# qiujiaming315/edgeml-object-detection

Hardware: AMD Instinct MI355X
Metric: images/sec/GPU at 640x640 (SSDLite & FRCNN-R50); ORIE max-abs-diff vs ref (higher is better)
Workload: dtype f32; 1 GPU; ssdlite320_mobilenet_v3_large b=32 640x640 (configs[1]); global_batch=32, parallelism=dp1, batches_in_flight=4, conv_math=bf16x6, weights=seeded synthetic (COCO weights need a download)

## Files before the change

### edgeml-object-detection_amd/csrc/layers.hip

```cpp
#include <cmath>
#include <cstdlib>
#include <mutex>
#include <type_traits>
#include <utility>
#include <vector>

#include "kernels.hpp"

namespace edgedet {



__device__ __forceinline__ float div_fast(float a, float b, float rb) {
    const float q = a * rb;
    return fmaf(fmaf(-q, b, a), rb, q);
}

template <typename T, bool FAST = false>
__device__ __forceinline__ float pre_load(const T* src, int64_t i) {
    if constexpr (sizeof(T) == 1) return FAST ? div_fast((float)src[i], 255.f, 1.f / 255.f) : (float)src[i] / 255.f;
    else return src[i];
}

template <typename T, bool FAST = false>
__device__ __forceinline__ f32x4 pre_pixel(const T* __restrict__ xb, int H, int W, float sh, float sw,
                                           const float* mean, const float* stdv, const float* rstd, int oy, int ox) {
    float ry = __builtin_fmaf(sh, (float)oy + 0.5f, -0.5f);
    float rx = __builtin_fmaf(sw, (float)ox + 0.5f, -0.5f);
    ry = ry < 0.f ? 0.f : ry;
    rx = rx < 0.f ? 0.f : rx;
    const int y0 = min((int)ry, H - 1), x0 = min((int)rx, W - 1);
    const int y1 = y0 + ((y0 < H - 1) ? 1 : 0);
    const int x1 = x0 + ((x0 < W - 1) ? 1 : 0);
    const float ly = fminf(fmaxf(ry - (float)y0, 0.f), 1.f), lx = fminf(fmaxf(rx - (float)x0, 0.f), 1.f);
    const float hy = 1.f - ly, hx = 1.f - lx;
    float v[3];
#pragma unroll
    for (int c = 0; c < 3; ++c) {
        const T* src = xb + (int64_t)c * H * W;
        auto norm = [&](int64_t i) {
            const float a = pre_load<T, FAST>(src, i) - mean[c];
            return FAST ? div_fast(a, stdv[c], rstd[c]) : a / stdv[c];
        };
        const float a00 = norm((int64_t)y0 * W + x0);
        const float a01 = norm((int64_t)y0 * W + x1);
        const float a10 = norm((int64_t)y1 * W + x0);
        const float a11 = norm((int64_t)y1 * W + x1);
        v[c] = __builtin_fmaf(__builtin_fmaf(a00, hx, a01 * lx), hy, __builtin_fmaf(a10, hx, a11 * lx) * ly);
    }
    return f32x4{v[0], v[1], v[2], 0.f};
}

static bool u8_fast_div(const float mean[3], const float stdv[3], float rstd[3]) {
    const float r255 = 1.f / 255.f;
    for (int c = 0; c < 3; ++c) rstd[c] = 1.f / stdv[c];
    auto same = [](float a, float b) { return __builtin_memcmp(&a, &b, sizeof(float)) == 0; };
    auto fast = [](float a, float b, float rb) {
        const float q = a * rb;
        return std::fma(std::fma(-q, b, a), rb, q);
    };
    for (int x = 0; x < 256; ++x) {
        const float xf = (float)x, t = xf / 255.f;
        if (!same(fast(xf, 255.f, r255), t)) return false;
        for (int c = 0; c < 3; ++c) {
            const float a = t - mean[c];
            if (!same(fast(a, stdv[c], rstd[c]), a / stdv[c])) return false;
        }
    }
    return true;
}

template <typename T, bool FAST>
__global__ void preprocess_kernel(PreParams p, const T* __restrict__ x) {
    const int64_t idx = (int64_t)blockIdx.x * blockDim.x + threadIdx.x;
    const int64_t total = (int64_t)p.B * p.Hp * p.Wp;
    if (idx >= total) return;
    const int ox = (int)(idx % p.Wp);
    const int oy = (int)((idx / p.Wp) % p.Hp);
    const int b = (int)(idx / ((int64_t)p.Wp * p.Hp));
    f32x4 out = {0.f, 0.f, 0.f, 0.f};
    if (oy < p.Ho && ox < p.Wo) out = pre_pixel<T, FAST>(x + (int64_t)b * 3 * p.H * p.W, p.H, p.W, p.sh, p.sw, p.mean, p.stdv, p.rstd, oy, ox);
    *reinterpret_cast<f32x4*>(p.y + idx * 4) = out;
}

int preprocess_launch(const PreParams& p0, hipStream_t s) {
    PreParams p = p0;
    EDGEDET_REQUIRE(p.y && ((p.x != nullptr) != (p.xu8 != nullptr)), "preprocess: null y, or not exactly one of x (f32) / x (u8)");
    EDGEDET_REQUIRE(p.Hp >= p.Ho && p.Wp >= p.Wo && p.Ho > 0 && p.Wo > 0, "preprocess: bad sizes");
    p.sh = (float)p.H / (float)p.Ho;
    p.sw = (float)p.W / (float)p.Wo;
    const int64_t total = (int64_t)p.B * p.Hp * p.Wp;
    p.fastdiv = p.xu8 && u8_fast_div(p.mean, p.stdv, p.rstd);
    if (p.xu8) {
        void (*k)(PreParams, const uint8_t*) = p.fastdiv ? preprocess_kernel<uint8_t, true> : preprocess_kernel<uint8_t, false>;
        hipLaunchKernelGGL(k, dim3((unsigned)cdiv(total, 256)), dim3(256), 0, s, p, p.xu8);
    } else {
        void (*k)(PreParams, const float*) = preprocess_kernel<float, false>;
        hipLaunchKernelGGL(k, dim3((unsigned)cdiv(total, 256)), dim3(256), 0, s, p, p.x);
    }
    EDGEDET_LAUNCH_CHECK();
    return 0;
}


__global__ void dwconv_kernel(DwParams p) {
    const int C4 = p.C >> 2;
    const int64_t idx = (int64_t)blockIdx.x * blockDim.x + threadIdx.x;
    const int64_t total = (int64_t)p.B * p.Ho * p.Wo * C4;
    if (idx >= total) return;
    const int c = (int)(idx % C4) * 4;
    const int64_t pix = idx / C4;
    const int ow = (int)(pix % p.Wo);
    const int oh = (int)((pix / p.Wo) % p.Ho);
    const int b = (int)(pix / ((int64_t)p.Wo * p.Ho));
    const float* xb = p.x + (int64_t)b * p.H * p.W * p.C + c;
    f32x4 acc = {0.f, 0.f, 0.f, 0.f};
    const int ih0 = oh * p.stride - p.pad, iw0 = ow * p.stride - p.pad;
    for (int kh = 0; kh < p.K; ++kh) {
        const int ih = ih0 + kh;
        if ((unsigned)ih >= (unsigned)p.H) continue;
        for (int kw = 0; kw < p.K; ++kw) {
            const int iw = iw0 + kw;
            if ((unsigned)iw >= (unsigned)p.W) continue;
            const f32x4 xv = *reinterpret_cast<const f32x4*>(xb + ((int64_t)ih * p.W + iw) * p.C);
            const f32x4 wv = *reinterpret_cast<const f32x4*>(p.w + (kh * p.K + kw) * p.C + c);
            acc.x = fmaf(xv.x, wv.x, acc.x);
            acc.y = fmaf(xv.y, wv.y, acc.y);
            acc.z = fmaf(xv.z, wv.z, acc.z);
            acc.w = fmaf(xv.w, wv.w, acc.w);
        }
    }
    const f32x4 bv = *reinterpret_cast<const f32x4*>(p.bias + c);
    f32x4 o;
    o.x = apply_act(acc.x + bv.x, p.act);
    o.y = apply_act(acc.y + bv.y, p.act);
    o.z = apply_act(acc.z + bv.z, p.act);
    o.w = apply_act(acc.w + bv.w, p.act);
    *reinterpret_cast<f32x4*>(p.y + pix * p.C + c) = o;
}

__global__ void __launch_bounds__(256) dwconv_se_kernel(DwParams p) {
    __shared__ f32x4 red[16][16];
    const int cq = threadIdx.x & 15, pl = threadIdx.x >> 4;
    const int c = blockIdx.x * 64 + cq * 4;
    const int sidx = blockIdx.y, b = blockIdx.z;
    const int HWo = p.Ho * p.Wo;
    const int p0 = (int)((int64_t)sidx * HWo / p.parts), p1 = (int)((int64_t)(sidx + 1) * HWo / p.parts);
    f32x4 sum = {0.f, 0.f, 0.f, 0.f};
    if (c < p.C) {
        const float* xb = p.x + (int64_t)b * p.H * p.W * p.C + c;
        const f32x4 bv = *reinterpret_cast<const f32x4*>(p.bias + c);
        for (int pix = p0 + pl; pix < p1; pix += 16) {
            const int oh = pix / p.Wo, ow = pix - oh * p.Wo;
            const int ih0 = oh * p.stride - p.pad, iw0 = ow * p.stride - p.pad;
            f32x4 acc = {0.f, 0.f, 0.f, 0.f};
            for (int kh = 0; kh < p.K; ++kh) {
                const int ih = ih0 + kh;
                if ((unsigned)ih >= (unsigned)p.H) continue;
                for (int kw = 0; kw < p.K; ++kw) {
                    const int iw = iw0 + kw;
                    if ((unsigned)iw >= (unsigned)p.W) continue;
                    const f32x4 xv = *reinterpret_cast<const f32x4*>(xb + ((int64_t)ih * p.W + iw) * p.C);
                    const f32x4 wv = *reinterpret_cast<const f32x4*>(p.w + (kh * p.K + kw) * p.C + c);
                    acc.x = fmaf(xv.x, wv.x, acc.x);
                    acc.y = fmaf(xv.y, wv.y, acc.y);
                    acc.z = fmaf(xv.z, wv.z, acc.z);
                    acc.w = fmaf(xv.w, wv.w, acc.w);
                }
            }
            f32x4 o;
            o.x = apply_act(acc.x + bv.x, p.act);
            o.y = apply_act(acc.y + bv.y, p.act);
            o.z = apply_act(acc.z + bv.z, p.act);
            o.w = apply_act(acc.w + bv.w, p.act);
            *reinterpret_cast<f32x4*>(p.y + ((int64_t)b * HWo + pix) * p.C + c) = o;
            sum += o;
        }
    }
    red[pl][cq] = sum;
    __syncthreads();
    if (pl == 0 && c < p.C) {
        f32x4 t = red[0][cq];
        for (int q = 1; q < 16; ++q) t += red[q][cq];
        *reinterpret_cast<f32x4*>(p.part + ((int64_t)b * p.parts + sidx) * p.C + c) = t;
    }
}

template <int K, int S>
constexpr int dw_rows() {
    return K == 5 && S == 2 ? 2 : 3;
}

template <int K, int S, int PW>
__device__ __forceinline__ void dw_cols(const DwParams& p, uint32_t lane, int iw0, uint32_t (&co)[(PW - 1) * S + K]) {
    const int cb = p.C * 4, hi = (p.W - 1) * cb;
    int o = iw0 * cb;
#pragma unroll
    for (int j = 0; j < (PW - 1) * S + K; ++j, o += cb) co[j] = lane + (uint32_t)min(max(o, 0), hi);
}

template <int K, int S, int PW>
__device__ __forceinline__ void dw_load_row(const DwParams& p, const float* __restrict__ base,
                                            const uint32_t (&co)[(PW - 1) * S + K], int ih,
                                            f32x4 (&x)[(PW - 1) * S + K]) {
    const uint32_t ro = (uint32_t)(min(max(ih, 0), p.H - 1) * p.W) * (uint32_t)(p.C * 4);
#pragma unroll
    for (int j = 0; j < (PW - 1) * S + K; ++j)
        x[j] = *reinterpret_cast<const f32x4*>(reinterpret_cast<const char*>(base) + (co[j] + ro));
}

template <int K, int S, int PW, typename WF>
__device__ __forceinline__ void dw_fma_row(const DwParams& p, int ih, int iw0, f32x4 (&x)[(PW - 1) * S + K], WF w,
                                           f32x4 (&acc)[PW]) {
    const bool rin = (unsigned)ih < (unsigned)p.H;
#pragma unroll
    for (int j = 0; j < (PW - 1) * S + K; ++j)
        x[j] = rin && (unsigned)(iw0 + j) < (unsigned)p.W ? x[j] : f32x4{0.f, 0.f, 0.f, 0.f};
    f32x4 wv[K];
#pragma unroll
    for (int kw = 0; kw < K; ++kw) wv[kw] = w(kw);
#pragma unroll
    for (int kw = 0; kw < K; ++kw)
#pragma unroll
        for (int o = 0; o < PW; ++o) acc[o] = __builtin_elementwise_fma(x[o * S + kw], wv[kw], acc[o]);
}

template <int PW, bool SUM, typename AF>
__device__ __forceinline__ void dw_store(const DwParams& p, float* yb, int ow0, const f32x4 (&acc)[PW],
                                         const f32x4& bv, f32x4& sum, AF af) {
#pragma unroll
    for (int o = 0; o < PW; ++o) {
        if (ow0 + o < p.Wo) {
            f32x4 v;
            v.x = af(acc[o].x + bv.x);
            v.y = af(acc[o].y + bv.y);
            v.z = af(acc[o].z + bv.z);
            v.w = af(acc[o].w + bv.w);
            *reinterpret_cast<f32x4*>(yb + (int64_t)o * p.C) = v;
            if (SUM) sum += v;
        }
    }
}

template <int PW, bool SUM>
__device__ __forceinline__ void dw_finish(const DwParams& p, float* yb, int ow0, const f32x4 (&acc)[PW],
                                          const f32x4& bv, f32x4& sum) {
    const int act = p.act;
    if (act == ACT_HSWISH)
        dw_store<PW, SUM>(p, yb, ow0, acc, bv, sum, [](float v) { return apply_act(v, ACT_HSWISH); });
    else if (act == ACT_RELU)
        dw_store<PW, SUM>(p, yb, ow0, acc, bv, sum, [](float v) { return apply_act(v, ACT_RELU); });
    else if (act == ACT_NONE)
        dw_store<PW, SUM>(p, yb, ow0, acc, bv, sum, [](float v) { return apply_act(v, ACT_NONE); });
    else
        dw_store<PW, SUM>(p, yb, ow0, acc, bv, sum, [act](float v) { return apply_act(v, act); });
}

template <int K, int S, int PW>
__device__ __forceinline__ void dwconv_rb_body(const DwParams& p, int nq, int nwg, int64_t idx) {
    constexpr int IW = (PW - 1) * S + K;
    const int64_t total = (int64_t)p.B * p.Ho * nwg * nq;
    if (idx >= total) return;
    int q, wg, oh, b;
    if (total <= 0x7fffffff) {
        const uint32_t i = (uint32_t)idx, r0 = i / (uint32_t)nq, r1 = r0 / (uint32_t)nwg;
        q = (int)(i - r0 * (uint32_t)nq);
        wg = (int)(r0 - r1 * (uint32_t)nwg);
        b = (int)(r1 / (uint32_t)p.Ho);
        oh = (int)(r1 - (uint32_t)b * (uint32_t)p.Ho);
    } else {
        q = (int)(idx % nq);
        int64_t r = idx / nq;
        wg = (int)(r % nwg);
        r /= nwg;
        oh = (int)(r % p.Ho);
        b = (int)(r / p.Ho);
    }
    constexpr int R = dw_rows<K, S>();
    const int c = q * 4, ow0 = wg * PW;
    const int ih0 = oh * S - p.pad, iw0 = ow0 * S - p.pad;
    const float* wq = p.w + c;
    uint32_t co[IW];
    dw_cols<K, S, PW>(p, ((uint32_t)(b * p.H * p.W) * (uint32_t)p.C + (uint32_t)c) * 4u, iw0, co);
    f32x4 buf[R][IW], wr[R][K], acc[PW];
#pragma unroll
    for (int r = 0; r < R; ++r) {
        dw_load_row<K, S, PW>(p, p.x, co, ih0 + r, buf[r]);
#pragma unroll
        for (int kw = 0; kw < K; ++kw) wr[r][kw] = *reinterpret_cast<const f32x4*>(wq + (r * K + kw) * p.C);
    }
    const f32x4 bv = *reinterpret_cast<const f32x4*>(p.bias + c);
#pragma unroll
    for (int o = 0; o < PW; ++o) acc[o] = f32x4{0.f, 0.f, 0.f, 0.f};
#pragma unroll
    for (int kh = 0; kh < K; ++kh) {
        const int sl = kh % R;
        dw_fma_row<K, S, PW>(p, ih0 + kh, iw0, buf[sl], [&](int kw) { return wr[sl][kw]; }, acc);
        if (kh + R < K) {
            dw_load_row<K, S, PW>(p, p.x, co, ih0 + kh + R, buf[sl]);
#pragma unroll
            for (int kw = 0; kw < K; ++kw)
                wr[sl][kw] = *reinterpret_cast<const f32x4*>(wq + ((kh + R) * K + kw) * p.C);
        }
    }
    f32x4 unused;
    dw_finish<PW, false>(p, p.y + (((int64_t)b * p.Ho + oh) * p.Wo + ow0) * p.C + c, ow0, acc, bv, unused);
}

template <int K, int S, int PW>
__global__ void __launch_bounds__(256) dwconv_rb_kernel(DwParams p, int nq, int nwg) {
    dwconv_rb_body<K, S, PW>(p, nq, nwg, (int64_t)blockIdx.x * blockDim.x + threadIdx.x);
}

template <int K, int S, int PW>
__global__ void __launch_bounds__(256) dwconv_rb_group_kernel(DwGroup g) {
    const int bx = (int)blockIdx.x;
    int k = 0;
    while (k + 1 < g.n && bx >= g.start[k + 1]) ++k;
    dwconv_rb_body<K, S, PW>(g.p[k], g.nq[k], g.nwg[k], (int64_t)(bx - g.start[k]) * blockDim.x + threadIdx.x);
}

template <int K, int S>
constexpr int dw_se_waves() {
    return K == 3 && S == 2 ? 2 : 3;
}

template <int K, int S, int PW, int QL = 16>
__global__ void __launch_bounds__(256, (dw_se_waves<K, S>())) dwconv_rb_se_kernel(DwParams p, int nq, int nwg) {
    constexpr int GL = 256 / QL;
    constexpr int IW = (PW - 1) * S + K, R = dw_rows<K, S>();
    __shared__ f32x4 red[GL][QL];
    constexpr int WU = ((K * K + 1) * QL + 255) / 256;
    __shared__ f32x4 wl[WU * GL][QL];
    const int ql = threadIdx.x % QL, gl = threadIdx.x / QL;
    const int q = blockIdx.x * QL + ql;
    const int c = q * 4;
    const int sidx = blockIdx.y, b = blockIdx.z;
    const int G = p.Ho * nwg;
    const int g0 = (int)((int64_t)sidx * G / p.parts), g1 = (int)((int64_t)(sidx + 1) * G / p.parts);
    const bool live = q < nq;
    const int cl = live ? c : (nq - 1) * 4;
    const float* xb = p.x + (int64_t)b * p.H * p.W * p.C;
    f32x4 sum = {0.f, 0.f, 0.f, 0.f};
    f32x4 buf[R][IW];
    int g = g0 + gl;
    if (live && g < g1) {
        const int oh = g / nwg, ow0 = (g - oh * nwg) * PW;
        uint32_t co[IW];
        dw_cols<K, S, PW>(p, (uint32_t)cl * 4u, ow0 * S - p.pad, co);
#pragma unroll
        for (int r = 0; r < R; ++r) dw_load_row<K, S, PW>(p, xb, co, oh * S - p.pad + r, buf[r]);
    }
    {
        f32x4 wv[WU];
        const int tq = min(q, nq - 1) * 4;
#pragma unroll
        for (int u = 0; u < WU; ++u) {
            const int t = gl + u * GL;
            wv[u] = *reinterpret_cast<const f32x4*>((t < K * K ? p.w + t * p.C : p.bias) + tq);
        }
#pragma unroll
        for (int u = 0; u < WU; ++u) wl[gl + u * GL][ql] = wv[u];
    }
    __syncthreads();
    auto pass = [&](auto more) {
        constexpr bool MORE = decltype(more)::value;
        const int oh = g / nwg, ow0 = (g - oh * nwg) * PW;
        const int ih0 = oh * S - p.pad, iw0 = ow0 * S - p.pad;
        const int gn = g + GL;
        const int ohn = gn / nwg, ih0n = ohn * S - p.pad, iw0n = (gn - ohn * nwg) * PW * S - p.pad;
        int qv = ql;
        asm volatile("" : "+v"(qv));
        f32x4 acc[PW];
#pragma unroll
        for (int o = 0; o < PW; ++o) acc[o] = f32x4{0.f, 0.f, 0.f, 0.f};
#pragma unroll
        for (int kh = 0; kh < K; ++kh) {
            const int sl = kh % R;
            dw_fma_row<K, S, PW>(p, ih0 + kh, iw0, buf[sl], [&](int kw) { return wl[kh * K + kw][qv]; }, acc);
            if (kh + R < K || MORE) {
                const bool own = kh + R < K;
                uint32_t co[IW];
                dw_cols<K, S, PW>(p, (uint32_t)cl * 4u, own ? iw0 : iw0n, co);
                dw_load_row<K, S, PW>(p, xb, co, own ? ih0 + kh + R : ih0n + sl, buf[sl]);
            }
        }
        dw_finish<PW, true>(p, p.y + (((int64_t)b * p.Ho + oh) * p.Wo + ow0) * p.C + c, ow0, acc, wl[K * K][qv], sum);
        g = gn;
    };
    if (live && g < g1) {
        while (g + GL < g1) pass(std::true_type{});
        pass(std::false_type{});
    }
    red[gl][ql] = sum;
    __syncthreads();
    if (gl == 0 && live) {
        f32x4 t = red[0][ql];
        for (int k = 1; k < GL; ++k) t += red[k][ql];
        *reinterpret_cast<f32x4*>(p.part + ((int64_t)b * p.parts + sidx) * p.C + c) = t;
    }
}

static bool dw_offsets_fit(const DwParams& p) { return (int64_t)p.B * p.H * p.W * p.C * 4 < (1ll << 31); }

template <int K, int S>
static int dwconv_rb_launch(const DwParams& p, hipStream_t s) {
    constexpr int PW = 4;
    const int nq = p.C / 4, nwg = cdiv(p.Wo, PW);
    if (p.part) {
        hipLaunchKernelGGL((dwconv_rb_se_kernel<K, S, PW>), dim3((unsigned)cdiv(nq, 16), p.parts, p.B), dim3(256), 0,
                           s, p, nq, nwg);
    } else {
        const int64_t total = (int64_t)p.B * p.Ho * nwg * nq;
        hipLaunchKernelGGL((dwconv_rb_kernel<K, S, PW>), dim3((unsigned)cdiv(total, 256)), dim3(256), 0, s, p, nq,
                           nwg);
    }
    EDGEDET_LAUNCH_CHECK();
    return 0;
}

constexpr int STEM_T = 16, STEM_SH = STEM_T + 2, STEM_XH = 2 * STEM_SH + 1, STEM_SS = 20;
constexpr int STEM_W0 = 0, STEM_B0 = 576, STEM_WD = 592, STEM_BD = 736, STEM_W1 = 752, STEM_B1 = 1008, STEM_NW = 1024;

template <typename T, bool FUSED, bool FAST = false>
__global__ void __launch_bounds__(256) ssd_stem_kernel(StemParams p, int tiles_w) {
    __shared__ __attribute__((aligned(16))) float xs[STEM_XH * STEM_XH * 4];
    __shared__ __attribute__((aligned(16))) float ss[STEM_SH * STEM_SH * STEM_SS];
    __shared__ __attribute__((aligned(16))) float ws[STEM_NW];
    const int tid = threadIdx.x, b = blockIdx.y;
    const int oh0 = (blockIdx.x / tiles_w) * STEM_T, ow0 = (blockIdx.x % tiles_w) * STEM_T;
    const int sh0 = oh0 - 1, sw0 = ow0 - 1;
    const int xh0 = 2 * sh0 - 1, xw0 = 2 * sw0 - 1;
    const float* xb = FUSED ? nullptr : p.x + (int64_t)b * p.H * p.W * 4;
    {
        float wv[STEM_NW / 256];
#pragma unroll
        for (int r = 0; r < STEM_NW / 256; ++r) {
            const int e = tid + 256 * r;
            const float* src = e < STEM_B0   ? p.w0 + (e / 36) * p.ld0 + e % 36
                               : e < STEM_WD ? p.b0 + (e - STEM_B0)
                               : e < STEM_BD ? p.wd + (e - STEM_WD)
                               : e < STEM_W1 ? p.bd + (e - STEM_BD)
                               : e < STEM_B1 ? p.w1 + ((e - STEM_W1) / 16) * p.ld1 + (e - STEM_W1) % 16
                                             : p.b1 + (e - STEM_B1);
            wv[r] = *src;
        }
        constexpr int R = (STEM_XH * STEM_XH + 255) / 256;
        f32x4 xv[R];
#pragma unroll
        for (int r = 0; r < R; ++r) {
            const int v = tid + 256 * r;
            const int ih = xh0 + v / STEM_XH, iw = xw0 + v % STEM_XH;
            const bool in = v < STEM_XH * STEM_XH && (unsigned)ih < (unsigned)p.H && (unsigned)iw < (unsigned)p.W;
            if constexpr (FUSED) {
                const T* img = (const T*)(sizeof(T) == 1 ? (const void*)p.src8 : (const void*)p.src) +
                               (int64_t)b * 3 * p.H0 * p.W0;
                xv[r] = in ? pre_pixel<T, FAST>(img, p.H0, p.W0, p.sh, p.sw, p.mean, p.stdv, p.rstd, ih, iw)
                           : f32x4{0.f, 0.f, 0.f, 0.f};
            } else {
                const float* src = xb + (in ? ((int64_t)ih * p.W + iw) * 4 : 0);
                xv[r] = *reinterpret_cast<const f32x4*>(src);
                if (!in) xv[r] = f32x4{0.f, 0.f, 0.f, 0.f};
            }
        }
#pragma unroll
        for (int r = 0; r < R; ++r)
            if (tid + 256 * r < STEM_XH * STEM_XH) *reinterpret_cast<f32x4*>(xs + 4 * (tid + 256 * r)) = xv[r];
#pragma unroll
        for (int r = 0; r < STEM_NW / 256; ++r) ws[tid + 256 * r] = wv[r];
    }
    __syncthreads();
    const int lane = tid & 63, wid = tid >> 6, l16 = lane & 15, q4 = lane >> 4;
    float wb[9];
#pragma unroll
    for (int t = 0; t < 9; ++t) wb[t] = ws[STEM_W0 + l16 * 36 + 4 * t + q4];
    const float b0v = ws[STEM_B0 + l16];
    constexpr int NV = STEM_SH * STEM_SH, NTL = (NV + 15) / 16;
    for (int tl = wid; tl < NTL; tl += 4) {
        const int va = min(16 * tl + l16, NV - 1);
        const int lh = va / STEM_SH, lw = va - lh * STEM_SH;
        f32x4 acc = {0.f, 0.f, 0.f, 0.f};
#pragma unroll
        for (int t = 0; t < 9; ++t) {
            const float av = xs[4 * ((2 * lh + t / 3) * STEM_XH + 2 * lw + t % 3) + q4];
            acc = __builtin_amdgcn_mfma_f32_16x16x4f32(av, wb[t], acc, 0, 0, 0);
        }
#pragma unroll
        for (int i = 0; i < 4; ++i) {
            const int v = 16 * tl + 4 * q4 + i;
            if (v < NV) {
                const int vh = v / STEM_SH, vw = v - vh * STEM_SH;
                const bool in = (unsigned)(sh0 + vh) < (unsigned)p.Ho && (unsigned)(sw0 + vw) < (unsigned)p.Wo;
                ss[v * STEM_SS + l16] = in ? apply_act(acc[i] + b0v, ACT_HSWISH) : 0.f;
            }
        }
    }
    __syncthreads();
    const int lh = tid / STEM_T, lw = tid % STEM_T;
    const int oh = oh0 + lh, ow = ow0 + lw;
    float dv[16];
#pragma unroll
    for (int c = 0; c < 16; ++c) dv[c] = 0.f;
#pragma unroll
    for (int kh = 0; kh < 3; ++kh) {
        if ((unsigned)(oh - 1 + kh) >= (unsigned)p.Ho) continue;
#pragma unroll
        for (int kw = 0; kw < 3; ++kw) {
            const float* sv = ss + ((lh + kh) * STEM_SH + lw + kw) * STEM_SS;
            const float* wv = ws + STEM_WD + (kh * 3 + kw) * 16;
#pragma unroll
            for (int c = 0; c < 16; ++c) dv[c] = fmaf(sv[c], wv[c], dv[c]);
        }
    }
    constexpr int DS = 17;
    float* dsm = xs;
#pragma unroll
    for (int c = 0; c < 16; ++c) dsm[tid * DS + c] = apply_act(dv[c] + ws[STEM_BD + c], ACT_RELU);
    float w1v[4];
#pragma unroll
    for (int k = 0; k < 4; ++k) w1v[k] = ws[STEM_W1 + l16 * 16 + 4 * k + q4];
    const float b1v = ws[STEM_B1 + l16];
    __syncthreads();
#pragma unroll
    for (int tl = 0; tl < 4; ++tl) {
        const int row0 = 64 * wid + 16 * tl;
        f32x4 acc = {0.f, 0.f, 0.f, 0.f};
#pragma unroll
        for (int k = 0; k < 4; ++k)
            acc = __builtin_amdgcn_mfma_f32_16x16x4f32(dsm[(row0 + l16) * DS + 4 * k + q4], w1v[k], acc, 0, 0, 0);
#pragma unroll
        for (int i = 0; i < 4; ++i) {
            const int px = row0 + 4 * q4 + i, ph = px / STEM_T, pw = px % STEM_T;
            const int yh = oh0 + ph, yw = ow0 + pw;
            if (yh < p.Ho && yw < p.Wo) {
                const float r = ss[((ph + 1) * STEM_SH + pw + 1) * STEM_SS + l16];
                p.y[(((int64_t)b * p.Ho + yh) * p.Wo + yw) * 16 + l16] = (acc[i] + b1v) + r;
            }
        }
    }
}

int ssd_stem_launch(const StemParams& p0, hipStream_t s) {
    StemParams p = p0;
    const bool fused = p.src || p.src8;
    EDGEDET_REQUIRE((p.x || fused) && p.w0 && p.b0 && p.wd && p.bd && p.w1 && p.b1 && p.y, "ssd_stem: null pointer");
    EDGEDET_REQUIRE(!(p.src && p.src8), "ssd_stem: one source image (float or uint8)");
    if (fused) {
        EDGEDET_REQUIRE(p.H0 >= 1 && p.W0 >= 1, "ssd_stem: source image size");
        p.sh = (float)p.H0 / (float)p.H;
        p.sw = (float)p.W0 / (float)p.W;
    }
    EDGEDET_REQUIRE(p.Ho == (p.H - 1) / 2 + 1 && p.Wo == (p.W - 1) / 2 + 1, "ssd_stem: 3x3 stride 2 pad 1 shape");
    EDGEDET_REQUIRE(p.ld0 >= 36 && p.ld1 >= 16, "ssd_stem: weight row strides");
    const int tiles_w = cdiv(p.Wo, STEM_T);
    const dim3 grid((unsigned)(cdiv(p.Ho, STEM_T) * tiles_w), (unsigned)p.B);
    p.fastdiv = p.src8 && u8_fast_div(p.mean, p.stdv, p.rstd);
    void (*k)(StemParams, int) = p.src8 ? (p.fastdiv ? ssd_stem_kernel<uint8_t, true, true> : ssd_stem_kernel<uint8_t, true>)
                                 : p.src ? ssd_stem_kernel<float, true> : ssd_stem_kernel<float, false>;
    hipLaunchKernelGGL(k, grid, dim3(256), 0, s, p, tiles_w);
    EDGEDET_LAUNCH_CHECK();
    return 0;
}

extern "C" int edgedet_ssd_stem(const float* x, int64_t B, int64_t H, int64_t W, const float* w0, int64_t ld0,
                                const float* b0, const float* wd, const float* bd, const float* w1, int64_t ld1,
                                const float* b1, float* y, void* stream) {
    StemParams p{};
    p.x = x;
    p.w0 = w0;
    p.b0 = b0;
    p.wd = wd;
    p.bd = bd;
    p.w1 = w1;
    p.b1 = b1;
    p.y = y;
    p.B = (int)B;
    p.H = (int)H;
    p.W = (int)W;
    p.Ho = (int)((H - 1) / 2 + 1);
    p.Wo = (int)((W - 1) / 2 + 1);
    p.ld0 = (int)ld0;
    p.ld1 = (int)ld1;
    return ssd_stem_launch(p, (hipStream_t)stream);
}

constexpr int MBW_C = 16;
constexpr int MBW_MAXW = 8;

template <int K, int S, int CINP, int TH, int TW>
struct MbwGeom {
    static constexpr int IHh = (TH - 1) * S + K, IWh = (TW - 1) * S + K;
    static constexpr int NPX = IHh * IWh, NPXP = (NPX + 15) / 16 * 16;
    static constexpr int P = TH * TW;
    static constexpr int XS = CINP + 1;
    static constexpr int ES = MBW_C + 1;
    static constexpr int PS = 33;
    static constexpr int EW = NPXP * ES > P * PS ? NPXP * ES : P * PS;
    static size_t smem(int nw) { return 4 * ((size_t)NPXP * (XS + 1) + (size_t)nw * (EW + P * ES)); }
};

__device__ __forceinline__ void mbw_lds_barrier() {
    asm volatile("s_waitcnt lgkmcnt(0)\n\ts_barrier" ::: "memory");
}

__device__ __forceinline__ void mbw_wave_sync() {
    __builtin_amdgcn_fence(__ATOMIC_RELEASE, "workgroup");
    __builtin_amdgcn_wave_barrier();
    __builtin_amdgcn_fence(__ATOMIC_ACQUIRE, "workgroup");
}

template <int K, int S, int ACT, int CINP, int TH, int TW>
__global__ void __launch_bounds__(64 * MBW_MAXW, 4) mbconv_kernel(MbParams p, int tiles_w, int tiles_img, int ntiles) {
    using G = MbwGeom<K, S, CINP, TH, TW>;
    constexpr int IWh = G::IWh, NPX = G::NPX, NPXP = G::NPXP, P = G::P;
    constexpr int XS = G::XS, ES = G::ES, PS = G::PS, EW = G::EW;
    constexpr int NT = NPXP / 16, KS = CINP / 4, PT = P / 16, Q4 = CINP / 4;
    constexpr int HR = (NPXP * Q4 + 255) / 256;
    static_assert(P % 16 == 0 && TW % 4 == 0 && NPXP <= 256, "mbconv: tile shape");
    extern __shared__ __attribute__((aligned(16))) float mb_smem[];
    const int nt = (int)blockDim.x, nw = nt >> 6;
    const int tid = threadIdx.x, lane = tid & 63, wid = tid >> 6, l16 = lane & 15, q = lane >> 4;
    float* xs = mb_smem;
    float* es = mb_smem + NPXP * XS + wid * EW;
    float* ds = mb_smem + NPXP * XS + nw * EW + wid * P * ES;
    float* xm = mb_smem + NPXP * XS + nw * (EW + P * ES);
    const int Cin = p.Cin, Cexp = p.Cexp, Cout = p.Cout;
    const int ch = wid * MBW_C + l16;
    const bool chv = ch < Cexp;
    float w1r[KS], w2r[4][2], wdr[K * K];
    const int chc = chv ? ch : 0;
#pragma unroll
    for (int s = 0; s < KS; ++s) {
        const bool ok = chv && 4 * s + q < Cin;
        const float v = p.w1[(int64_t)chc * p.ld1 + (ok ? 4 * s + q : 0)];
        w1r[s] = ok ? v : 0.f;
    }
#pragma unroll
    for (int s = 0; s < 4; ++s)
#pragma unroll
        for (int n = 0; n < 2; ++n) {
            const int co = 16 * n + l16, k = wid * MBW_C + 4 * s + q;
            const bool ok = co < Cout && k < Cexp;
            const float v = p.w2[ok ? (int64_t)co * p.ld2 + k : 0];
            w2r[s][n] = ok ? v : 0.f;
        }
#pragma unroll
    for (int t = 0; t < K * K; ++t) {
        const float v = p.wd[(int64_t)t * Cexp + chc];
        wdr[t] = chv ? v : 0.f;
    }
    const float b1 = chv ? p.b1[chc] : 0.f, bd = chv ? p.bd[chc] : 0.f;
    const int co_t = tid & 31;
    const float b2v = p.b2[co_t < Cout ? co_t : 0];
    f32x4 hv[HR];
    int hr[HR], hc[HR], hoff[HR], hdst[HR];
#pragma unroll
    for (int u = 0; u < HR; ++u) {
        const int t = tid + nt * u, px = t / Q4, c4 = t - px * Q4;
        const bool live = t < NPXP * Q4 && px < NPX && 4 * c4 < Cin;
        hr[u] = live ? px / IWh : -(1 << 20);
        hc[u] = px % IWh;
        hoff[u] = 4 * c4;
        hdst[u] = t < NPXP * Q4 ? px * XS + 4 * c4 : -1;
    }
    const int mr = tid < NPXP ? tid / IWh : 0, mc = tid % IWh;
    uint32_t hok = 0;
    auto load_halo = [&](int tile) {
        const int b = tile / tiles_img, r = tile - b * tiles_img, th = r / tiles_w, tw = r - th * tiles_w;
        const int ih0 = th * TH * S - p.pad, iw0 = tw * TW * S - p.pad;
        const float* xb = p.x + (int64_t)b * p.H * p.W * Cin;
#pragma unroll
        for (int u = 0; u < HR; ++u) {
            const int ih = ih0 + hr[u], iw = iw0 + hc[u];
            const bool ok = (unsigned)ih < (unsigned)p.H && (unsigned)iw < (unsigned)p.W;
            const int off = ((ih * p.W + iw) * Cin + hoff[u]) * (int)ok;
            hv[u] = *reinterpret_cast<const f32x4*>(xb + off);
            hok = (hok & ~(1u << u)) | ((uint32_t)ok << u);
        }
    };
    int tile = blockIdx.x;
    if (tile < ntiles) load_halo(tile);
    for (; tile < ntiles; tile += gridDim.x) {
        const int b = tile / tiles_img, r = tile - b * tiles_img, th = r / tiles_w, tw = r - th * tiles_w;
        const int oh0 = th * TH, ow0 = tw * TW, ih0 = oh0 * S - p.pad, iw0 = ow0 * S - p.pad;
        mbw_lds_barrier();
#pragma unroll
        for (int u = 0; u < HR; ++u) {
            if (hdst[u] >= 0) {
                const f32x4 v = (hok >> u) & 1 ? hv[u] : f32x4{0.f, 0.f, 0.f, 0.f};
                float* d = xs + hdst[u];
                d[0] = v.x;
                d[1] = v.y;
                d[2] = v.z;
                d[3] = v.w;
            }
        }
        if (tid < NPXP) {
            const int ih = ih0 + mr, iw = iw0 + mc;
            xm[tid] = tid < NPX && (unsigned)ih < (unsigned)p.H && (unsigned)iw < (unsigned)p.W ? 1.f : 0.f;
        }
        if (tile + (int)gridDim.x < ntiles) load_halo(tile + gridDim.x);
        mbw_lds_barrier();
        auto expand_store = [&](const f32x4& a, int t) {
#pragma unroll
            for (int i = 0; i < 4; ++i) {
                const int m = 16 * t + 4 * q + i;
                es[m * ES + l16] = apply_act(a[i] + b1, ACT) * xm[m];
            }
        };
#pragma unroll 1
        for (int t = 0; t < NT; t += 2) {
            f32x4 a0 = {0.f, 0.f, 0.f, 0.f}, a1 = {0.f, 0.f, 0.f, 0.f};
            const float* r0 = xs + (16 * t + l16) * XS + q;
#pragma unroll
            for (int s = 0; s < KS; ++s) {
                a0 = __builtin_amdgcn_mfma_f32_16x16x4f32(r0[4 * s], w1r[s], a0, 0, 0, 0);
                if (t + 1 < NT) a1 = __builtin_amdgcn_mfma_f32_16x16x4f32(r0[16 * XS + 4 * s], w1r[s], a1, 0, 0, 0);
            }
            expand_store(a0, t);
            if (t + 1 < NT) expand_store(a1, t + 1);
        }
        mbw_wave_sync();
#pragma unroll 1
        for (int oy = q; oy < TH; oy += 4) {
            float win[K][K];
#pragma unroll
            for (int kh = 0; kh < K; ++kh)
#pragma unroll
                for (int kw = 0; kw < K; ++kw) win[kh][kw] = es[((oy * S + kh) * IWh + kw) * ES + l16];
#pragma unroll
            for (int ox = 0; ox < TW; ++ox) {
                if (ox > 0) {
#pragma unroll
                    for (int kh = 0; kh < K; ++kh) {
#pragma unroll
                        for (int kw = 0; kw < K - S; ++kw) win[kh][kw] = win[kh][kw + S];
#pragma unroll
                        for (int kw = K - S; kw < K; ++kw)
                            win[kh][kw] = es[((oy * S + kh) * IWh + ox * S + kw) * ES + l16];
                    }
                }
                float a = 0.f;
#pragma unroll
                for (int kh = 0; kh < K; ++kh)
#pragma unroll
                    for (int kw = 0; kw < K; ++kw) a = fmaf(win[kh][kw], wdr[kh * K + kw], a);
                ds[(oy * TW + ox) * ES + l16] = apply_act(a + bd, ACT);
            }
        }
        mbw_wave_sync();
        f32x4 acc[PT][2];
#pragma unroll
        for (int t = 0; t < PT; ++t) acc[t][0] = acc[t][1] = f32x4{0.f, 0.f, 0.f, 0.f};
#pragma unroll
        for (int s = 0; s < 4; ++s)
#pragma unroll
            for (int t = 0; t < PT; ++t) {
                const float a = ds[(16 * t + l16) * ES + 4 * s + q];
                acc[t][0] = __builtin_amdgcn_mfma_f32_16x16x4f32(a, w2r[s][0], acc[t][0], 0, 0, 0);
                acc[t][1] = __builtin_amdgcn_mfma_f32_16x16x4f32(a, w2r[s][1], acc[t][1], 0, 0, 0);
            }
#pragma unroll
        for (int t = 0; t < PT; ++t)
#pragma unroll
            for (int n = 0; n < 2; ++n)
#pragma unroll
                for (int i = 0; i < 4; ++i) es[(16 * t + 4 * q + i) * PS + 16 * n + l16] = acc[t][n][i];
        mbw_lds_barrier();
        const float* part = mb_smem + NPXP * XS;
        for (int e = tid; e < P * 32; e += nt) {
            const int px = e >> 5, co = e & 31;
            const int ly = px / TW, lx = px - ly * TW, oh = oh0 + ly, ow = ow0 + lx;
            if (co >= Cout || oh >= p.Ho || ow >= p.Wo) continue;
            float v = part[px * PS + co];
            for (int w = 1; w < nw; ++w) v += part[w * EW + px * PS + co];
            v += b2v;
            if (p.residual) v += xs[((ly + p.pad) * IWh + lx + p.pad) * XS + co];
            p.y[(((int64_t)b * p.Ho + oh) * p.Wo + ow) * Cout + co] = v;
        }
    }
}

template <typename KF>
static int mbw_set_lds(KF kernel, size_t bytes) {
    static std::mutex mu;
    static std::vector<std::pair<const void*, size_t>> done;
    std::lock_guard<std::mutex> lk(mu);
    for (auto& d : done)
        if (d.first == (const void*)kernel && d.second >= bytes) return 0;
    EDGEDET_CHECK_HIP(hipFuncSetAttribute((const void*)kernel, hipFuncAttributeMaxDynamicSharedMemorySize, (int)bytes));
    done.emplace_back((const void*)kernel, bytes);
    return 0;
}

template <int K, int S, int ACT, int CINP>
static int mbconv_launch_t(const MbParams& p, hipStream_t s) {
    constexpr int TH = S == 1 ? 8 : 4, TW = 8;
    using G = MbwGeom<K, S, CINP, TH, TW>;
    const int nw = std::max(4, (int)cdiv(p.Cexp, MBW_C)), tiles_w = (int)cdiv(p.Wo, TW);
    const int tiles_img = (int)cdiv(p.Ho, TH) * tiles_w, ntiles = p.B * tiles_img;
    const size_t lds = G::smem(nw);
    EDGEDET_REQUIRE(lds <= 160 * 1024, "mbconv: tile exceeds the LDS");
    auto kern = mbconv_kernel<K, S, ACT, CINP, TH, TW>;
    if (int rc = mbw_set_lds(kern, lds)) return rc;
    const int per_cu = std::max(1, (int)((160 * 1024) / lds));
    const int grid = std::min(ntiles, 256 * per_cu);
    hipLaunchKernelGGL(kern, dim3((unsigned)grid), dim3(64 * nw), lds, s, p, tiles_w, tiles_img, ntiles);
    EDGEDET_LAUNCH_CHECK();
    return 0;
}

template <int K, int S, int ACT>
static int mbconv_launch_a(const MbParams& p, hipStream_t s) {
    if (p.Cin <= 16) return mbconv_launch_t<K, S, ACT, 16>(p, s);
    if (p.Cin <= 24) return mbconv_launch_t<K, S, ACT, 24>(p, s);
    return mbconv_launch_t<K, S, ACT, 32>(p, s);
}

template <int K, int S>
static int mbconv_launch_ks(const MbParams& p, hipStream_t s) {
    switch (p.act) {
        case ACT_RELU: return mbconv_launch_a<K, S, ACT_RELU>(p, s);
        case ACT_RELU6: return mbconv_launch_a<K, S, ACT_RELU6>(p, s);
        case ACT_HSWISH: return mbconv_launch_a<K, S, ACT_HSWISH>(p, s);
        default: EDGEDET_REQUIRE(false, "mbconv: activation RE / R6 / HS");
    }
}

int mbconv_launch(const MbParams& p, hipStream_t s) {
    EDGEDET_REQUIRE(p.x && p.w1 && p.b1 && p.wd && p.bd && p.w2 && p.b2 && p.y, "mbconv: null pointer");
    EDGEDET_REQUIRE(p.Cin >= 1 && p.Cin <= 32 && p.Cin % 4 == 0 && p.Cout >= 1 && p.Cout <= 32 && p.Cexp >= 1 &&
                        p.Cexp <= MBW_C * MBW_MAXW,
                    "mbconv: Cin <= 32 (a multiple of 4), Cout <= 32, Cexp <= 128");
    EDGEDET_REQUIRE(((uintptr_t)p.x & 15) == 0, "mbconv: input 16-byte aligned");
    EDGEDET_REQUIRE(p.ld1 >= p.Cin && p.ld2 >= p.Cexp, "mbconv: weight row strides");
    EDGEDET_REQUIRE(p.pad == (p.K - 1) / 2 && p.Ho == (p.H + 2 * p.pad - p.K) / p.stride + 1 &&
                    p.Wo == (p.W + 2 * p.pad - p.K) / p.stride + 1, "mbconv: 'same' padding shape");
    EDGEDET_REQUIRE(!p.residual || (p.stride == 1 && p.Cin == p.Cout), "mbconv: residual needs stride 1, Cin == Cout");
    if (p.K == 3 && p.stride == 1) return mbconv_launch_ks<3, 1>(p, s);
    if (p.K == 3 && p.stride == 2) return mbconv_launch_ks<3, 2>(p, s);
    if (p.K == 5 && p.stride == 1) return mbconv_launch_ks<5, 1>(p, s);
    if (p.K == 5 && p.stride == 2) return mbconv_launch_ks<5, 2>(p, s);
    EDGEDET_REQUIRE(false, "mbconv: K in {3, 5}, stride in {1, 2}");
}

int dwconv_group_launch(const DwParams* ps, int n, hipStream_t s) {
    EDGEDET_REQUIRE(n >= 1 && n <= EDGEDET_MAX_GROUP, "dwconv group: 1..EDGEDET_MAX_GROUP members");
    constexpr int PW = 4;
    DwGroup g;
    g.n = n;
    const int K = ps[0].K, S = ps[0].stride;
// ... 528 lines not shown
```

Measured before the change: 33600 images/s.

## Restructure SSD stem LDS layout and precompute resize coordinates per tile

The fused stem kernel now computes bilinear resize coordinates once per tile row and column into a shared table instead of per pixel. It stores the input tile in a planar, even/odd-split LDS layout so the stride-2 conv reads are bank-friendly and a zero pad slot replaces the fourth channel. Tap loads are issued before any arithmetic to overlap memory latency, and boundary masks and address tables are precomputed. The output epilogue uses simpler per-wave addressing. Costs are extra LDS use, more code complexity, and a new 31-bit limit on source image size.

Result: faster. 34140 images/s (median of 6 runs) (+1.6%).

```diff
diff --git a/edgeml-object-detection_amd/csrc/layers.hip b/edgeml-object-detection_amd/csrc/layers.hip
--- a/edgeml-object-detection_amd/csrc/layers.hip
+++ b/edgeml-object-detection_amd/csrc/layers.hip
@@ -17,38 +17,70 @@
 }
 
 template <typename T, bool FAST = false>
-__device__ __forceinline__ float pre_load(const T* src, int64_t i) {
-    if constexpr (sizeof(T) == 1) return FAST ? div_fast((float)src[i], 255.f, 1.f / 255.f) : (float)src[i] / 255.f;
-    else return src[i];
-}
-
-template <typename T, bool FAST = false>
-__device__ __forceinline__ f32x4 pre_pixel(const T* __restrict__ xb, int H, int W, float sh, float sw,
-                                           const float* mean, const float* stdv, const float* rstd, int oy, int ox) {
+__device__ __forceinline__ float pre_load(T raw) {
+    if constexpr (sizeof(T) == 1) return FAST ? div_fast((float)raw, 255.f, 1.f / 255.f) : (float)raw / 255.f;
+    else return raw;
+}
+
+struct PreCoord {
+    int y0, y1, x0, x1;
+    float ly, lx;
+};
+
+__device__ __forceinline__ PreCoord pre_coord(int H, int W, float sh, float sw, int oy, int ox) {
     float ry = __builtin_fmaf(sh, (float)oy + 0.5f, -0.5f);
     float rx = __builtin_fmaf(sw, (float)ox + 0.5f, -0.5f);
     ry = ry < 0.f ? 0.f : ry;
     rx = rx < 0.f ? 0.f : rx;
-    const int y0 = min((int)ry, H - 1), x0 = min((int)rx, W - 1);
-    const int y1 = y0 + ((y0 < H - 1) ? 1 : 0);
-    const int x1 = x0 + ((x0 < W - 1) ? 1 : 0);
-    const float ly = fminf(fmaxf(ry - (float)y0, 0.f), 1.f), lx = fminf(fmaxf(rx - (float)x0, 0.f), 1.f);
+    PreCoord k;
+    k.y0 = min((int)ry, H - 1);
+    k.x0 = min((int)rx, W - 1);
+    k.y1 = k.y0 + ((k.y0 < H - 1) ? 1 : 0);
+    k.x1 = k.x0 + ((k.x0 < W - 1) ? 1 : 0);
+    k.ly = fminf(fmaxf(ry - (float)k.y0, 0.f), 1.f);
+    k.lx = fminf(fmaxf(rx - (float)k.x0, 0.f), 1.f);
+    return k;
+}
+
+template <typename T, typename I>
+__device__ __forceinline__ void pre_taps(const T* __restrict__ xb, I plane, const I (&o)[4], T (&raw)[12]) {
+#pragma unroll
+    for (int c = 0; c < 3; ++c) {
+        const T* src = xb + (I)c * plane;
+#pragma unroll
+        for (int t = 0; t < 4; ++t) raw[4 * c + t] = src[o[t]];
+    }
+}
+
+template <typename T, bool FAST = false>
+__device__ __forceinline__ f32x4 pre_value(const T (&raw)[12], float ly, float lx, const float* mean, const float* stdv,
+                                           const float* rstd) {
     const float hy = 1.f - ly, hx = 1.f - lx;
     float v[3];
 #pragma unroll
     for (int c = 0; c < 3; ++c) {
-        const T* src = xb + (int64_t)c * H * W;
-        auto norm = [&](int64_t i) {
-            const float a = pre_load<T, FAST>(src, i) - mean[c];
+        auto norm = [&](T r) {
+            const float a = pre_load<T, FAST>(r) - mean[c];
             return FAST ? div_fast(a, stdv[c], rstd[c]) : a / stdv[c];
         };
-        const float a00 = norm((int64_t)y0 * W + x0);
-        const float a01 = norm((int64_t)y0 * W + x1);
-        const float a10 = norm((int64_t)y1 * W + x0);
-        const float a11 = norm((int64_t)y1 * W + x1);
+        const float a00 = norm(raw[4 * c]);
+        const float a01 = norm(raw[4 * c + 1]);
+        const float a10 = norm(raw[4 * c + 2]);
+        const float a11 = norm(raw[4 * c + 3]);
         v[c] = __builtin_fmaf(__builtin_fmaf(a00, hx, a01 * lx), hy, __builtin_fmaf(a10, hx, a11 * lx) * ly);
     }
     return f32x4{v[0], v[1], v[2], 0.f};
+}
+
+template <typename T, bool FAST = false>
+__device__ __forceinline__ f32x4 pre_pixel(const T* __restrict__ xb, int H, int W, float sh, float sw,
+                                           const float* mean, const float* stdv, const float* rstd, int oy, int ox) {
+    const PreCoord k = pre_coord(H, W, sh, sw, oy, ox);
+    const int64_t o[4] = {(int64_t)k.y0 * W + k.x0, (int64_t)k.y0 * W + k.x1, (int64_t)k.y1 * W + k.x0,
+                          (int64_t)k.y1 * W + k.x1};
+    T raw[12];
+    pre_taps<T, int64_t>(xb, (int64_t)H * W, o, raw);
+    return pre_value<T, FAST>(raw, k.ly, k.lx, mean, stdv, rstd);
 }
 
 static bool u8_fast_div(const float mean[3], const float stdv[3], float rstd[3]) {
@@ -421,53 +453,105 @@
 
 constexpr int STEM_T = 16, STEM_SH = STEM_T + 2, STEM_XH = 2 * STEM_SH + 1, STEM_SS = 20;
 constexpr int STEM_W0 = 0, STEM_B0 = 576, STEM_WD = 592, STEM_BD = 736, STEM_W1 = 752, STEM_B1 = 1008, STEM_NW = 1024;
+constexpr int STEM_RP = 41, STEM_ODD = 19, STEM_XP = 1520, STEM_XZ = 3 * STEM_XP, STEM_NZ = 104;
+constexpr int STEM_NV = STEM_SH * STEM_SH, STEM_NTL = (STEM_NV + 15) / 16, STEM_NVP = 16 * STEM_NTL;
+static_assert(STEM_XH * STEM_RP <= STEM_XP && 2 * STEM_RP + STEM_ODD < STEM_NZ && STEM_XZ >= 256 * 17, "stem LDS layout");
 
 template <typename T, bool FUSED, bool FAST = false>
 __global__ void __launch_bounds__(256) ssd_stem_kernel(StemParams p, int tiles_w) {
-    __shared__ __attribute__((aligned(16))) float xs[STEM_XH * STEM_XH * 4];
+    __shared__ __attribute__((aligned(16))) float xs[STEM_XZ + STEM_NZ];
     __shared__ __attribute__((aligned(16))) float ss[STEM_SH * STEM_SH * STEM_SS];
     __shared__ __attribute__((aligned(16))) float ws[STEM_NW];
+    __shared__ __attribute__((aligned(16))) uint32_t msk[STEM_NVP];
+    __shared__ int atab[STEM_NVP];
     const int tid = threadIdx.x, b = blockIdx.y;
     const int oh0 = (blockIdx.x / tiles_w) * STEM_T, ow0 = (blockIdx.x % tiles_w) * STEM_T;
     const int sh0 = oh0 - 1, sw0 = ow0 - 1;
     const int xh0 = 2 * sh0 - 1, xw0 = 2 * sw0 - 1;
     const float* xb = FUSED ? nullptr : p.x + (int64_t)b * p.H * p.W * 4;
     {
+        constexpr int NX = STEM_XH * STEM_XH, R = (NX + 255) / 256;
+        constexpr int STEM_OUT = 1 << 29;
+        [[maybe_unused]] int4* ct = reinterpret_cast<int4*>(ss);
+        if constexpr (FUSED) {
+            if (tid < 2 * STEM_XH) {
+                const bool isrow = tid < STEM_XH;
+                const int i = isrow ? tid : tid - STEM_XH;
+                const int g = (isrow ? xh0 : xw0) + i, n = isrow ? p.H : p.W, gc = min(max(g, 0), n - 1);
+                const PreCoord k = pre_coord(p.H0, p.W0, p.sh, p.sw, gc, gc);
+                const int place = (isrow ? i * STEM_RP : (i & 1) * STEM_ODD + (i >> 1)) + ((unsigned)g < (unsigned)n ? 0 : STEM_OUT);
+                ct[tid] = isrow ? make_int4(k.y0 * p.W0, k.y1 * p.W0, __float_as_int(k.ly), place)
+                                : make_int4(k.x0, k.x1, __float_as_int(k.lx), place);
+            }
+            __syncthreads();
+        }
         float wv[STEM_NW / 256];
+        __builtin_assume(tid >= 0 && tid < 256);
 #pragma unroll
         for (int r = 0; r < STEM_NW / 256; ++r) {
-            const int e = tid + 256 * r;
-            const float* src = e < STEM_B0   ? p.w0 + (e / 36) * p.ld0 + e % 36
-                               : e < STEM_WD ? p.b0 + (e - STEM_B0)
-                               : e < STEM_BD ? p.wd + (e - STEM_WD)
-                               : e < STEM_W1 ? p.bd + (e - STEM_BD)
-                               : e < STEM_B1 ? p.w1 + ((e - STEM_W1) / 16) * p.ld1 + (e - STEM_W1) % 16
-                                             : p.b1 + (e - STEM_B1);
-            wv[r] = *src;
-        }
-        constexpr int R = (STEM_XH * STEM_XH + 255) / 256;
+            const int e = tid + 256 * r, e1 = max(e - STEM_W1, 0);
+            const int o_w1 = (e1 >> 4) * p.ld1 + (e1 & 15), o_w0 = (e / 36) * p.ld0 + e % 36;
+            const int o_bd = e - STEM_BD, o_wd = e - STEM_WD, o_b0 = e - STEM_B0;
+            const bool c_w1 = r >= STEM_W1 / 256 && e < STEM_B1, c_bd = r == STEM_W1 / 256 && e < STEM_W1;
+            const bool c_wd = r == STEM_BD / 256 && e < STEM_BD, c_b0 = r == STEM_WD / 256 && e < STEM_WD;
+            const bool c_w0 = r <= STEM_B0 / 256 && e < STEM_B0;
+            const float* base = p.b1;
+            int off = e - STEM_B1;
+            base = c_w1 ? p.w1 : base, off = c_w1 ? o_w1 : off;
+            base = c_bd ? p.bd : base, off = c_bd ? o_bd : off;
+            base = c_wd ? p.wd : base, off = c_wd ? o_wd : off;
+            base = c_b0 ? p.b0 : base, off = c_b0 ? o_b0 : off;
+            base = c_w0 ? p.w0 : base, off = c_w0 ? o_w0 : off;
+            wv[r] = base[off];
+        }
+        int xi[R];
+        bool inb[R];
+        [[maybe_unused]] float ly[R], lx[R];
+        [[maybe_unused]] T raw[R][12];
         f32x4 xv[R];
 #pragma unroll
         for (int r = 0; r < R; ++r) {
-            const int v = tid + 256 * r;
-            const int ih = xh0 + v / STEM_XH, iw = xw0 + v % STEM_XH;
-            const bool in = v < STEM_XH * STEM_XH && (unsigned)ih < (unsigned)p.H && (unsigned)iw < (unsigned)p.W;
+            const int v = min(tid + 256 * r, NX - 1);
+            const int row = v / STEM_XH, col = v - row * STEM_XH;
             if constexpr (FUSED) {
                 const T* img = (const T*)(sizeof(T) == 1 ? (const void*)p.src8 : (const void*)p.src) +
                                (int64_t)b * 3 * p.H0 * p.W0;
-                xv[r] = in ? pre_pixel<T, FAST>(img, p.H0, p.W0, p.sh, p.sw, p.mean, p.stdv, p.rstd, ih, iw)
-                           : f32x4{0.f, 0.f, 0.f, 0.f};
+                const int4 ky = ct[row], kx = ct[STEM_XH + col];
+                const uint32_t o[4] = {(uint32_t)(ky.x + kx.x), (uint32_t)(ky.x + kx.y), (uint32_t)(ky.y + kx.x),
+                                       (uint32_t)(ky.y + kx.y)};
+                pre_taps<T, uint32_t>(img, (uint32_t)(p.H0 * p.W0), o, raw[r]);
+                ly[r] = __int_as_float(ky.z);
+                lx[r] = __int_as_float(kx.z);
+                inb[r] = ky.w + kx.w < STEM_OUT;
+                xi[r] = (ky.w + kx.w) & (STEM_OUT - 1);
             } else {
-                const float* src = xb + (in ? ((int64_t)ih * p.W + iw) * 4 : 0);
-                xv[r] = *reinterpret_cast<const f32x4*>(src);
-                if (!in) xv[r] = f32x4{0.f, 0.f, 0.f, 0.f};
+                const int ih = xh0 + row, iw = xw0 + col;
+                inb[r] = (unsigned)ih < (unsigned)p.H && (unsigned)iw < (unsigned)p.W;
+                xi[r] = row * STEM_RP + (col & 1) * STEM_ODD + (col >> 1);
+                const float* src = xb + (inb[r] ? ((int64_t)ih * p.W + iw) * 4 : 0);
+                xv[r] = f32x4{src[0], src[1], src[2], 0.f};
             }
         }
-#pragma unroll
-        for (int r = 0; r < R; ++r)
-            if (tid + 256 * r < STEM_XH * STEM_XH) *reinterpret_cast<f32x4*>(xs + 4 * (tid + 256 * r)) = xv[r];
+        __builtin_amdgcn_sched_barrier(0);
+#pragma unroll
+        for (int r = 0; r < (STEM_NVP + 255) / 256; ++r) {
+            const int e = tid + 256 * r;
+            if (e < STEM_NVP) {
+                const int v = min(e, STEM_NV - 1), vh = v / STEM_SH, vw = v - vh * STEM_SH;
+                const bool in = e < STEM_NV && (unsigned)(sh0 + vh) < (unsigned)p.Ho && (unsigned)(sw0 + vw) < (unsigned)p.Wo;
+                msk[e] = in ? 0xffffffffu : 0u;
+                atab[e] = 2 * vh * STEM_RP + vw;
+            }
+        }
+        if (tid < STEM_NZ) xs[STEM_XZ + tid] = 0.f;
 #pragma unroll
         for (int r = 0; r < STEM_NW / 256; ++r) ws[tid + 256 * r] = wv[r];
+#pragma unroll
+        for (int r = 0; r < R; ++r) {
+            if constexpr (FUSED) xv[r] = pre_value<T, FAST>(raw[r], ly[r], lx[r], p.mean, p.stdv, p.rstd);
+#pragma unroll
+            for (int c = 0; c < 3; ++c) xs[c * STEM_XP + xi[r]] = inb[r] ? xv[r][c] : 0.f;
+        }
     }
     __syncthreads();
     const int lane = tid & 63, wid = tid >> 6, l16 = lane & 15, q4 = lane >> 4;
@@ -475,35 +559,37 @@
 #pragma unroll
     for (int t = 0; t < 9; ++t) wb[t] = ws[STEM_W0 + l16 * 36 + 4 * t + q4];
     const float b0v = ws[STEM_B0 + l16];
-    constexpr int NV = STEM_SH * STEM_SH, NTL = (NV + 15) / 16;
-    for (int tl = wid; tl < NTL; tl += 4) {
-        const int va = min(16 * tl + l16, NV - 1);
-        const int lh = va / STEM_SH, lw = va - lh * STEM_SH;
+    constexpr int NJ = (STEM_NTL + 3) / 4;
+    int a0[NJ];
+#pragma unroll
+    for (int j = 0; j < NJ; ++j)
+        a0[j] = q4 == 3 ? STEM_XZ : atab[16 * min(wid + 4 * j, STEM_NTL - 1) + l16] + q4 * STEM_XP;
+#pragma unroll
+    for (int j = 0; j < NJ; ++j) {
+        const int tl = wid + 4 * j;
+        if (tl >= STEM_NTL) break;
         f32x4 acc = {0.f, 0.f, 0.f, 0.f};
 #pragma unroll
         for (int t = 0; t < 9; ++t) {
-            const float av = xs[4 * ((2 * lh + t / 3) * STEM_XH + 2 * lw + t % 3) + q4];
+            const float av = xs[a0[j] + (t / 3) * STEM_RP + (t % 3 == 1 ? STEM_ODD : t % 3 / 2)];
             acc = __builtin_amdgcn_mfma_f32_16x16x4f32(av, wb[t], acc, 0, 0, 0);
         }
-#pragma unroll
-        for (int i = 0; i < 4; ++i) {
-            const int v = 16 * tl + 4 * q4 + i;
-            if (v < NV) {
-                const int vh = v / STEM_SH, vw = v - vh * STEM_SH;
-                const bool in = (unsigned)(sh0 + vh) < (unsigned)p.Ho && (unsigned)(sw0 + vw) < (unsigned)p.Wo;
-                ss[v * STEM_SS + l16] = in ? apply_act(acc[i] + b0v, ACT_HSWISH) : 0.f;
-            }
+        const int v0 = 16 * tl + 4 * q4;
+        if (v0 < STEM_NV) {
+            const uint4 m = *reinterpret_cast<const uint4*>(msk + v0);
+            const uint32_t mi[4] = {m.x, m.y, m.z, m.w};
+#pragma unroll
+            for (int i = 0; i < 4; ++i)
+                ss[(v0 + i) * STEM_SS + l16] = __uint_as_float(__float_as_uint(apply_act(acc[i] + b0v, ACT_HSWISH)) & mi[i]);
         }
     }
     __syncthreads();
     const int lh = tid / STEM_T, lw = tid % STEM_T;
-    const int oh = oh0 + lh, ow = ow0 + lw;
     float dv[16];
 #pragma unroll
     for (int c = 0; c < 16; ++c) dv[c] = 0.f;
 #pragma unroll
     for (int kh = 0; kh < 3; ++kh) {
-        if ((unsigned)(oh - 1 + kh) >= (unsigned)p.Ho) continue;
 #pragma unroll
         for (int kw = 0; kw < 3; ++kw) {
             const float* sv = ss + ((lh + kh) * STEM_SH + lw + kw) * STEM_SS;
@@ -520,6 +606,13 @@
 #pragma unroll
     for (int k = 0; k < 4; ++k) w1v[k] = ws[STEM_W1 + l16 * 16 + 4 * k + q4];
     const float b1v = ws[STEM_B1 + l16];
+    const int wu = __builtin_amdgcn_readfirstlane(wid);
+    float* yb = p.y + (((int64_t)b * p.Ho + oh0 + 4 * wu) * p.Wo + ow0) * 16;
+    const float* rs = ss + ((4 * wid + 1) * STEM_SH + 4 * q4 + 1) * STEM_SS + l16;
+    const uint32_t yl = (uint32_t)(4 * q4 * 16 + l16);
+    bool okw[4];
+#pragma unroll
+    for (int i = 0; i < 4; ++i) okw[i] = ow0 + 4 * q4 + i < p.Wo;
     __syncthreads();
 #pragma unroll
     for (int tl = 0; tl < 4; ++tl) {
@@ -528,14 +621,15 @@
 #pragma unroll
         for (int k = 0; k < 4; ++k)
             acc = __builtin_amdgcn_mfma_f32_16x16x4f32(dsm[(row0 + l16) * DS + 4 * k + q4], w1v[k], acc, 0, 0, 0);
+        float r[4];
+#pragma unroll
+        for (int i = 0; i < 4; ++i) r[i] = rs[(tl * STEM_SH + i) * STEM_SS];
+        const bool okh = oh0 + 4 * wu + tl < p.Ho;
+        float* yt = yb + (int64_t)tl * p.Wo * 16;
 #pragma unroll
         for (int i = 0; i < 4; ++i) {
-            const int px = row0 + 4 * q4 + i, ph = px / STEM_T, pw = px % STEM_T;
-            const int yh = oh0 + ph, yw = ow0 + pw;
-            if (yh < p.Ho && yw < p.Wo) {
-                const float r = ss[((ph + 1) * STEM_SH + pw + 1) * STEM_SS + l16];
-                p.y[(((int64_t)b * p.Ho + yh) * p.Wo + yw) * 16 + l16] = (acc[i] + b1v) + r;
-            }
+            const float o = (acc[i] + b1v) + r[i];
+            if (okh && okw[i]) yt[yl + 16 * i] = o;
         }
     }
 }
@@ -547,6 +641,7 @@
     EDGEDET_REQUIRE(!(p.src && p.src8), "ssd_stem: one source image (float or uint8)");
     if (fused) {
         EDGEDET_REQUIRE(p.H0 >= 1 && p.W0 >= 1, "ssd_stem: source image size");
+        EDGEDET_REQUIRE(3 * (int64_t)p.H0 * p.W0 < ((int64_t)1 << 31), "ssd_stem: source image too large (3 H0 W0 must fit 31 bits)");
         p.sh = (float)p.H0 / (float)p.H;
         p.sw = (float)p.W0 / (float)p.W;
     }
```
